# gaozhihan/PreDiff

Hardware: AMD Instinct MI355X
Metric: denoising_steps_per_sec (higher is better)
Workload: dtype bf16; 1 GPU; SEVIR-LR 7->6 x128x128 (latent 13x16x16, C 256/512, depth [4,4], axial), DDIM-50 eta=0, no knowledge alignment (BASELINE.json configs[1]); trajectories_per_gpu=64, global_trajectories=64, sampler=ddim50, hip_graph=True, lanes=2, trajectories_per_launch=32, parallelism=ensemble-shard x1

## Files before the change

### prediff_amd/csrc/igemm.hip

```cpp
#include <type_traits>
#include "common.h"
#include "igemm_epilogue.h"

namespace PD_NS {

__device__ __attribute__((aligned(64))) uint32_t g_pd_zero_page[32];

#ifndef PD_BIG_TILE_DEFAULT
#define PD_BIG_TILE_DEFAULT 1
#endif

#define BLDS16(rsrc, ldsptr, voff, soff) \
  __builtin_amdgcn_raw_ptr_buffer_load_lds((rsrc), (__attribute__((address_space(3))) void*)(ldsptr), 16, (voff), (soff), 0, 0)
#define PD_OOB 0xffffff00u

template <int N>
__device__ __forceinline__ void wait_vmcnt() {
  asm volatile("s_waitcnt vmcnt(%0)" ::"n"(N) : "memory");
}

template <int BM, int BN, int BK, int NS, bool SPLIT, int KIND, int OCC = 2, int ESLAB = 1>
__global__ void __launch_bounds__(256, OCC) igemm_kernel(const pd_igemm_args p) {
#if defined(__HIP_DEVICE_COMPILE__)
  constexpr int ROWB = BK * 2;
  constexpr int CPR = ROWB / 16;
  constexpr int RPI = 256 / CPR;
  constexpr int A_TILE = BM * ROWB;
  constexpr int B_TILE = BN * ROWB;
  constexpr int NP = SPLIT ? 2 : 1;
  constexpr int STAGE = (A_TILE + B_TILE) * NP;
  constexpr int AI = BM / RPI, BI = BN / RPI;
  constexpr int LPS = (AI + BI) * NP;
  constexpr int KSUB = BK / 32;
  extern __shared__ __attribute__((aligned(16))) char smem[];

  const int tid = threadIdx.x;
  const int lane = tid & 63;
  const int wave = __builtin_amdgcn_readfirstlane(tid >> 6);

  const int tiles_n = (p.N + BN - 1) / BN;
  const int tiles_m = (p.M + BM - 1) / BM;
  const int nt = tiles_m * tiles_n;
  int t;
  {
    const int bid = blockIdx.x, xcd = bid & 7, q = nt >> 3, r = nt & 7;
    t = (xcd < r ? xcd * (q + 1) : r * (q + 1) + (xcd - r) * q) + (bid >> 3);
  }
  const int m0 = (t / tiles_n) * BM;
  const int n0 = (t % tiles_n) * BN;
  const int bz = blockIdx.z;

  const auto rA = __builtin_amdgcn_make_buffer_rsrc((void*)(p.A + (int64_t)bz * p.a_batch_stride), 0, p.a_bytes, 0x00020000);
  const auto rW = __builtin_amdgcn_make_buffer_rsrc((void*)(p.W + (int64_t)bz * p.w_batch_stride), 0, p.w_bytes, 0x00020000);
  const auto rAlo = __builtin_amdgcn_make_buffer_rsrc((void*)((SPLIT ? p.A_lo : p.A) + (int64_t)bz * p.a_batch_stride), 0, p.a_bytes, 0x00020000);
  const auto rWlo = __builtin_amdgcn_make_buffer_rsrc((void*)((SPLIT ? p.W_lo : p.W) + (int64_t)bz * p.w_batch_stride), 0, p.w_bytes, 0x00020000);

  const int srow = tid / CPR;
  const int spos = tid % CPR;
  const int schunk = (CPR == 8) ? (spos ^ ((srow >> 1) & 7)) : (spos ^ ((srow >> 2) & 3));
  int vt0[AI], vh0[AI], vw0[AI];
  uint32_t abase[AI];
  uint32_t aoff[AI];
#pragma unroll
  for (int i = 0; i < AI; ++i) {
    const int m = m0 + i * RPI + srow;
    if (KIND == 0) {
      aoff[i] = m < p.M ? ((uint32_t)m * (uint32_t)p.lda + schunk * 8) * 2u : PD_OOB;
    } else {
      const int hw_o = p.Ho * p.Wo, thw_o = p.To * hw_o;
      const bool ok = m < p.M;
      const int mm = ok ? m : 0;
      const int b = mm / thw_o, r1 = mm - b * thw_o;
      const int ot = r1 / hw_o, r2 = r1 - ot * hw_o;
      const int oh = r2 / p.Wo, ow = r2 - oh * p.Wo;
      vt0[i] = ok ? ot * p.st - p.pt : -(1 << 20);
      vh0[i] = oh * p.sh - p.ph;
      vw0[i] = ow * p.sw - p.pw;
      abase[i] = (uint32_t)b * (uint32_t)(p.Ti * p.Hi * p.Wi);
    }
  }
  uint32_t woff[BI];
#pragma unroll
  for (int i = 0; i < BI; ++i) {
    const int n = n0 + i * RPI + srow;
    woff[i] = n < p.N ? ((uint32_t)n * (uint32_t)p.ldw + schunk * 8) * 2u : PD_OOB;
  }
  const int kchunks = p.Cin / BK;
  const int nk = (p.debug_flags & 1) ? 0 : p.taps * kchunks;
  const int vT = p.vT > 0 ? p.vT : p.Ti * p.ut, vH = p.vH > 0 ? p.vH : p.Hi * p.uh, vW = p.vW > 0 ? p.vW : p.Wi * p.uw;
  const int khw = p.KH * p.KW;

  auto set_tap = [&](int tap) {
    if (p.w_fold > 0 && tap >= p.w_fold) tap -= p.w_fold;
    const int kt = tap / khw, r = tap - kt * khw;
    const int kh = r / p.KW, kw = r - kh * p.KW;
#pragma unroll
    for (int i = 0; i < AI; ++i) {
      const int vt = vt0[i] + kt, vh = vh0[i] + kh, vw = vw0[i] + kw;
      const bool ok = (unsigned)vt < (unsigned)vT && (unsigned)vh < (unsigned)vH && (unsigned)vw < (unsigned)vW;
      const int it = p.ut == 2 ? vt >> 1 : vt, ih = p.uh == 2 ? vh >> 1 : vh, iw = p.uw == 2 ? vw >> 1 : vw;
      aoff[i] = ok ? ((abase[i] + (uint32_t)((it * p.Hi + ih) * p.Wi + iw)) * (uint32_t)p.lda + schunk * 8) * 2u : PD_OOB;
    }
  };

  auto issue = [&](int stage, int ks) {
    const int tap = ks / kchunks, kc = ks - tap * kchunks;
    if (KIND != 0 && kc == 0) set_tap(tap);
    char* sbase = smem + stage * STAGE;
    const int ka = kc * (BK * 2);
    const int kw = (int)(((int64_t)tap * p.w_tap_stride + kc * BK) * 2);
#pragma unroll
    for (int i = 0; i < AI; ++i) {
      char* dst = sbase + (i * 256 + wave * 64) * 16;
      BLDS16(rA, dst, aoff[i], ka);
      if (SPLIT) BLDS16(rAlo, dst + A_TILE, aoff[i], ka);
    }
#pragma unroll
    for (int i = 0; i < BI; ++i) {
      char* dst = sbase + A_TILE * NP + (i * 256 + wave * 64) * 16;
      BLDS16(rW, dst, woff[i], kw);
      if (SPLIT) BLDS16(rWlo, dst + B_TILE, woff[i], kw);
    }
  };

  constexpr int TM16 = BM / 32, TN16 = BN / 32;
  f32x4 acc[TM16][TN16];
#pragma unroll
  for (int i = 0; i < TM16; ++i)
#pragma unroll
    for (int j = 0; j < TN16; ++j)
#pragma unroll
      for (int r = 0; r < 4; ++r) acc[i][j][r] = 0.f;

  const int wr = wave >> 1, wc = wave & 1;
  const int l16 = lane & 15, lg = lane >> 4;
  const int swz = (CPR == 8) ? ((l16 >> 1) & 7) : ((l16 >> 2) & 3);
  const int a_row_b = (wr * (BM / 2) + l16) * ROWB;
  const int b_row_b = (wc * (BN / 2) + l16) * ROWB;

  constexpr int D = NS - 1;
#pragma unroll
  for (int s0 = 0; s0 < D; ++s0)
    if (s0 < nk) issue(s0, s0);
  int stage = 0;
  for (int ks = 0; ks < nk; ++ks) {
    const int younger = min(D - 1, nk - ks - 1);
    if (D >= 3 && younger == 2) wait_vmcnt<2 * LPS>();
    else if (D >= 2 && younger == 1) wait_vmcnt<LPS>();
    else wait_vmcnt<0>();
    __builtin_amdgcn_s_barrier();
    if (ks + D < nk) issue((stage + D) % NS, ks + D);
    const char* sA = smem + stage * STAGE;
    const char* sB = sA + A_TILE * NP;
#pragma unroll
    for (int kk = 0; kk < KSUB; ++kk) {
      const int pos = ((kk * 4 + lg) ^ swz) * 16;
      op8 a[TM16], b[TN16], al[TM16], bl[TN16];
#pragma unroll
      for (int i = 0; i < TM16; ++i) {
        a[i] = *(const op8*)(sA + a_row_b + i * 16 * ROWB + pos);
        if (SPLIT) al[i] = *(const op8*)(sA + A_TILE + a_row_b + i * 16 * ROWB + pos);
      }
#pragma unroll
      for (int j = 0; j < TN16; ++j) {
        b[j] = *(const op8*)(sB + b_row_b + j * 16 * ROWB + pos);
        if (SPLIT) bl[j] = *(const op8*)(sB + B_TILE + b_row_b + j * 16 * ROWB + pos);
      }
#pragma unroll
      for (int i = 0; i < TM16; ++i)
#pragma unroll
        for (int j = 0; j < TN16; ++j) {
          if (SPLIT) {
            acc[i][j] = mfma_16x16x32(al[i], b[j], acc[i][j]);
            acc[i][j] = mfma_16x16x32(a[i], bl[j], acc[i][j]);
          }
          acc[i][j] = mfma_16x16x32(a[i], b[j], acc[i][j]);
        }
    }
    stage = stage + 1 == NS ? 0 : stage + 1;
  }

  constexpr int WM = BM / 2, WN = BN / 2;
  constexpr int WNS = WN / ESLAB;
  constexpr int TNS = TN16 / ESLAB;
  float* sC = (float*)smem + wave * (WM * WNS);
#pragma unroll
  for (int js = 0; js < ESLAB; ++js) {
    __syncthreads();
#pragma unroll
    for (int i = 0; i < TM16; ++i)
#pragma unroll
      for (int j = 0; j < TNS; ++j)
#pragma unroll
        for (int r = 0; r < 4; ++r)
          sC[(i * 16 + 4 * lg + r) * WNS + j * 16 + l16] = acc[i][js * TNS + j][r];
    __syncthreads();
    igemm_epilogue<WM, WNS>(p, sC, lane, m0 + wr * WM, p.M, n0 + wc * WN + js * WNS, bz);
  }
#endif
}

template <int BM, int BN, int BK, int NS, bool SPLIT, int KIND, int OCC = 2, int ESLAB = 1>
static int launch_igemm(const pd_igemm_args& a, hipStream_t s) {
  constexpr int stage = (BM + BN) * BK * 2 * (SPLIT ? 2 : 1);
  constexpr int epi = 4 * (BM / 2) * (BN / 2) * 4 / ESLAB;
  constexpr int lds = NS * stage > epi ? NS * stage : epi;
  static bool attr_set_dev[PD_MAX_DEVICES];
  bool& attr_set = attr_set_dev[pd_cur_device()];
  if (!attr_set) {
    hipError_t e = hipFuncSetAttribute((const void*)igemm_kernel<BM, BN, BK, NS, SPLIT, KIND, OCC, ESLAB>,
                                       hipFuncAttributeMaxDynamicSharedMemorySize, lds);
    if (e != hipSuccess) {
      pd_set_error("pd_igemm: hipFuncSetAttribute(%d) failed: %s", lds, hipGetErrorString(e));
      return PD_ERR_LAUNCH;
    }
    attr_set = true;
  }
  const int tiles = ((a.M + BM - 1) / BM) * ((a.N + BN - 1) / BN);
  dim3 grid(tiles, 1, a.nbatch > 0 ? a.nbatch : 1);
  hipLaunchKernelGGL((igemm_kernel<BM, BN, BK, NS, SPLIT, KIND, OCC, ESLAB>), grid, dim3(256), lds, s, a);
  PD_CHECK_LAUNCH();
  return PD_OK;
}

template <bool SPLIT, int KIND>
static int dispatch_igemm(const pd_igemm_args& a, int tile, hipStream_t s) {
  switch (tile) {
    case 1: return launch_igemm<128, 128, 64, 2, SPLIT, KIND>(a, s);
    case 2: return launch_igemm<64, 64, 64, 2, SPLIT, KIND>(a, s);
    case 3: return launch_igemm<128, 128, 32, 4, SPLIT, KIND>(a, s);
    case 4: return launch_igemm<128, 128, 64, 3, SPLIT, KIND>(a, s);
    case 5: return launch_igemm<128, 128, 32, 2, SPLIT, KIND, (SPLIT ? 2 : 4), 2>(a, s);
    case 6: return launch_igemm<128, 128, 32, 3, SPLIT, KIND, (SPLIT ? 2 : 3), 2>(a, s);
    case 8: return launch_igemm<128, 64, 64, 2, SPLIT, KIND>(a, s);
    case 9: return launch_igemm<64, 128, 64, 2, SPLIT, KIND>(a, s);
    default: pd_set_error("pd_igemm: unknown tile config %d", tile); return PD_ERR_ARG;
  }
}

bool pd_igemm256_supported(const pd_igemm_args& a, int kind);
int pd_igemm256_launch(const pd_igemm_args& a, int kind, hipStream_t s);

int pd_igemm256_ksplit(const pd_igemm_args& a, int kind);
int pd_igemm256_launch_splitk(const pd_igemm_args& a, int kind, hipStream_t s);

#if !PD_IS_F16
extern "C" int pd_f16_igemm(const pd_igemm_args*, pd_stream_t);
#endif

extern "C" int PD_ENTRY(igemm)(const pd_igemm_args* pa, pd_stream_t stream) {
  PD_CHECK_ARG(pa != nullptr, "pd_igemm: null args");
  PD_FORWARD_F16(pa->operand == PD_OPERAND_F16, pd_f16_igemm(pa, stream));
  pd_igemm_args a = *pa;
  PD_CHECK_ARG(!PD_IS_F16 || (!a.split && !a.fp8 && !a.out_bf16_lo), "pd_igemm: IEEE-half operands: no hi/lo split, no e4m3 operands");
  const int min_k_256 = a.min_k_256 > 0 ? a.min_k_256 : a.split ? 256 : 1024;
  PD_CHECK_ARG(a.A && a.W, "pd_igemm: A/W null");
  PD_CHECK_ARG(a.M > 0 && a.N > 0 && a.taps > 0, "pd_igemm: bad M/N/taps (%d,%d,%d)", a.M, a.N, a.taps);
  PD_CHECK_ARG(a.Cin > 0 && (a.Cin & 63) == 0, "pd_igemm: Cin=%d must be a positive multiple of 64 (zero padded)", a.Cin);
  PD_CHECK_ARG((a.lda & 7) == 0 && (a.ldw & 7) == 0, "pd_igemm: lda/ldw must be multiples of 8 (16 B rows)");
  PD_CHECK_ARG(a.w_fold >= 0 && (a.w_fold == 0 || (!a.split && !a.fp8 && a.taps == 2 * a.w_fold)),
               "pd_igemm: w_fold = %d needs taps = 2 w_fold (W_hi slabs then W_lo slabs), no hi/lo split, no e4m3 operands", a.w_fold);
  PD_CHECK_ARG((a.w_fold ? a.w_fold : a.taps) == a.KT * a.KH * a.KW, "pd_igemm: taps != KT*KH*KW");
  PD_CHECK_ARG((int64_t)a.B * a.To * a.Ho * a.Wo == a.M, "pd_igemm: M != B*To*Ho*Wo");
  PD_CHECK_ARG((a.ut == 1 || a.ut == 2) && (a.uh == 1 || a.uh == 2) && (a.uw == 1 || a.uw == 2), "pd_igemm: bad upsample");
  if (a.fp8) {
    PD_CHECK_ARG((a.Cin & 127) == 0 && (a.lda & 15) == 0 && (a.ldw & 15) == 0, "pd_igemm: fp8 operands need Cin %% 128 == 0 and lda/ldw %% 16 == 0");
    PD_CHECK_ARG(!a.split && a.nbatch <= 1, "pd_igemm: fp8 operands: no hi/lo split, no batch");
  }
  {
    const int eb = a.fp8 ? 1 : 2;
    const int64_t abytes = (int64_t)a.B * a.Ti * a.Hi * a.Wi * (int64_t)a.lda * eb;
    const int64_t wbytes = ((int64_t)(a.taps - 1) * a.w_tap_stride + (int64_t)a.N * a.ldw) * eb;
    PD_CHECK_ARG(abytes < 0xfffffe00ll && wbytes < 0xfffffe00ll, "pd_igemm: operand larger than a 4 GiB buffer descriptor");
    a.a_bytes = (uint32_t)abytes;
    a.w_bytes = (uint32_t)wbytes;
  }
  PD_CHECK_ARG(!a.split || (a.A_lo && a.W_lo), "pd_igemm: split needs A_lo and W_lo");
  PD_CHECK_ARG(!a.rowvec || a.rows_per_sample > 0, "pd_igemm: rowvec needs rows_per_sample");
  PD_CHECK_ARG(a.out_f32 || a.out_bf16, "pd_igemm: no output");
  hipStream_t s = (hipStream_t)stream;
  a.vec_epilogue = ((a.N & 3) == 0) && (!a.out_f32 || (a.ld_out & 3) == 0) && (!a.out_bf16 || (a.ld_outb & 3) == 0) &&
                   (!a.residual || (a.ld_res & 3) == 0) && (!a.rowvec || (a.ld_rowvec & 3) == 0) &&
                   (!a.mul || (a.ld_mul & 3) == 0) && (((uintptr_t)a.out_f32 | (uintptr_t)a.residual | (uintptr_t)a.rowvec |
                   (uintptr_t)a.mul) & 15) == 0 && (((uintptr_t)a.out_bf16 | (uintptr_t)a.out_bf16_lo) & 7) == 0 &&
                   ((a.out_batch_stride | a.outb_batch_stride | a.res_batch_stride) & 3) == 0;
  if (a.vec_epilogue && !a.out_f32 && a.out_bf16 && (a.N & 7) == 0 && (a.ld_outb & 7) == 0 && (a.outb_batch_stride & 7) == 0 &&
      (((uintptr_t)a.out_bf16 | (uintptr_t)a.out_bf16_lo) & 15) == 0)
    a.vec_epilogue = 2;
  if (a.out_fp8_log2 > 0) {
    PD_CHECK_ARG(a.vec_epilogue == 2 && !a.out_bf16_lo && !a.split && a.out_fp8_log2 <= 16,
                 "pd_igemm: an e4m3 output needs the 8-column vector epilogue (out_bf16 only, N %% 8 == 0, ld_outb %% 8 == 0, 16 B aligned), no split");
  }
  int tile = a.tile;
  const bool pointwise = (a.taps == 1 || a.w_fold == 1) && a.st == 1 && a.sh == 1 && a.sw == 1 && a.pt == 0 && a.ph == 0 && a.pw == 0 && a.ut == 1 &&
                         a.uh == 1 && a.uw == 1 && a.Ti == a.To && a.Hi == a.Ho && a.Wi == a.Wo && a.vT <= 0 && a.vH <= 0 && a.vW <= 0;
  const int kind = pointwise ? 0 : ((a.KT == 1 && a.Ti == 1 && a.To == 1) ? 1 : 2);
  a.ksplit = 1;
#if !PD_IS_F16
  if (a.fp8) {
    if (!pd_igemm256_supported(a, kind) || kind == 1) {
      pd_set_error("pd_igemm: fp8 operands are built for row-wise linear layers and stride-1, un-upsampled Conv3d launches only");
      return PD_ERR_UNSUPPORTED;
    }
    const int ks = (a.tile == 0 && !a.disable_256 && a.out_fp8_log2 <= 0) ? pd_igemm256_ksplit(a, kind) : 0;
    if (ks >= 2) {
      a.ksplit = ks;
      return pd_igemm256_launch_splitk(a, kind, s);
    }
    return pd_igemm256_launch(a, kind, s);
  }
#endif
  if (tile == 0 && !a.disable_256) {
    const int ks = pd_igemm256_ksplit(a, kind);
    if (ks >= 2) {
      a.ksplit = ks;
      return pd_igemm256_launch_splitk(a, kind, s);
    }
  }
  if (tile == 0) {
    const int64_t t128 = (int64_t)((a.M + 127) / 128) * ((a.N + 127) / 128) * (a.nbatch > 0 ? a.nbatch : 1);
    tile = t128 >= 192 ? ((!a.split && (int64_t)a.taps * a.Cin <= 256) ? 5 : PD_BIG_TILE_DEFAULT) : 2;
    if (tile == PD_BIG_TILE_DEFAULT && !a.disable_256 && (int64_t)a.taps * a.Cin >= min_k_256 && pd_igemm256_supported(a, kind)) {
      const int64_t t256 = (int64_t)((a.M + 255) / 256) * ((a.N + 255) / 256) * (a.nbatch > 0 ? a.nbatch : 1);
      const int64_t ncu = pd_num_cus();
      const int64_t r128 = a.split ? (t128 + ncu - 1) / ncu : (t128 + 2 * ncu - 1) / (2 * ncu), r256 = (t256 + ncu - 1) / ncu;
      if (a.split ? r256 * 11 <= r128 * 5 : r256 * 33 <= r128 * 20) tile = 7;
    }
  }
  if (a.split && tile == 4) tile = 1;
  if (tile == 7) {
    if (pd_igemm256_supported(a, kind)) return pd_igemm256_launch(a, kind, s);
    tile = PD_BIG_TILE_DEFAULT;
  }
#if !PD_IS_F16
  if (a.split) {
    if (kind == 0) return dispatch_igemm<true, 0>(a, tile, s);
    if (kind == 1) return dispatch_igemm<true, 1>(a, tile, s);
    return dispatch_igemm<true, 2>(a, tile, s);
  }
#endif
  if (kind == 0) return dispatch_igemm<false, 0>(a, tile, s);
  if (kind == 1) return dispatch_igemm<false, 1>(a, tile, s);
  return dispatch_igemm<false, 2>(a, tile, s);
}

}
```

Baseline: 1540 steps/s.

## Add halo-tiled 3x3x3 conv kernel reusing LDS frame tiles across spatial taps

```diff
diff --git a/prediff_amd/csrc/conv3d_halo.hip b/prediff_amd/csrc/conv3d_halo.hip
--- /dev/null
+++ b/prediff_amd/csrc/conv3d_halo.hip
@@ -0,0 +1,250 @@
+#include <algorithm>
+#include "common.h"
+#include "igemm_epilogue.h"
+
+namespace PD_NS {
+
+#define BLDS16(rsrc, ldsptr, voff, soff) \
+  __builtin_amdgcn_raw_ptr_buffer_load_lds((rsrc), (__attribute__((address_space(3))) void*)(ldsptr), 16, (voff), (soff), 0, 0)
+#define PD_OOB 0xffffff00u
+#define VMCNT(n) asm volatile("s_waitcnt vmcnt(" #n ")" ::: "memory")
+#define PHASE_SYNC()                   \
+  __builtin_amdgcn_sched_barrier(0);   \
+  __builtin_amdgcn_s_barrier();        \
+  __builtin_amdgcn_sched_barrier(0)
+
+namespace {
+constexpr int FW = 16;
+constexpr int HW = FW + 2;
+constexpr int HROWS = HW * HW;
+constexpr int PLROWS = 336;
+constexpr int PLANE = PLROWS * 16;
+constexpr int HALO = 8 * PLANE;
+constexpr int NPIECE = HALO / 1024;
+constexpr int WHT = 128 * 128;
+constexpr int WBUF = 2 * WHT;
+constexpr int W_OFF = 2 * HALO;
+constexpr int HALO_LDS = W_OFF + 2 * WBUF;
+static_assert(PLANE % 256 == 0 && HALO % 1024 == 0 && PLROWS >= HROWS, "halo plane layout");
+static_assert(HALO_LDS >= 8 * 128 * 32 * 4, "the epilogue stages 128 KB of accumulators in the operand buffers");
+
+struct FragH {
+  op8 v[2];
+};
+}
+
+__global__ void __launch_bounds__(512) conv3d_halo_kernel(const pd_igemm_args p) {
+#if defined(__HIP_DEVICE_COMPILE__)
+  extern __shared__ __attribute__((aligned(16))) char smem[];
+  const int tid = threadIdx.x;
+  const int lane = tid & 63;
+  const int wave = __builtin_amdgcn_readfirstlane(tid >> 6);
+  const int wr = wave >> 2, wc = wave & 3;
+
+  const int tiles_n = (p.N + 255) >> 8;
+  const int tiles_m = p.M >> 8;
+  const int nt = tiles_m * tiles_n;
+  int t;
+  {
+    const int bid = blockIdx.x, xcd = bid & 7, q = nt >> 3, r = nt & 7;
+    t = (xcd < r ? xcd * (q + 1) : r * (q + 1) + (xcd - r) * q) + (bid >> 3);
+  }
+  const int tm = t / tiles_n;
+  const int m0 = tm << 8;
+  const int n0 = (t % tiles_n) << 8;
+
+  const auto rA = __builtin_amdgcn_make_buffer_rsrc((void*)p.A, 0, p.a_bytes, 0x00020000);
+  const auto rW = __builtin_amdgcn_make_buffer_rsrc((void*)p.W, 0, p.w_bytes, 0x00020000);
+
+  const int srow = tid >> 3, spos = tid & 7;
+  const uint32_t w_sel = (uint32_t)(spos ^ ((srow >> 1) & 7)) * 16u;
+  uint32_t woff[2][2];
+#pragma unroll
+  for (int hh = 0; hh < 2; ++hh)
+#pragma unroll
+    for (int i = 0; i < 2; ++i) {
+      const int n = n0 + hh * 128 + i * 64 + srow;
+      woff[hh][i] = n < p.N ? ((uint32_t)n * (uint32_t)p.ldw) * 2u + w_sel : PD_OOB;
+    }
+  uint32_t hoff[6];
+#pragma unroll
+  for (int n = 0; n < 6; ++n) {
+    const int cell = (wave + 8 * n) * 64 + lane;
+    const int s = cell / PLROWS, r = cell - s * PLROWS;
+    const int hr = r / HW, hc = r - hr * HW;
+    const bool ok = cell < 8 * PLROWS && r < HROWS && hr >= 1 && hr <= FW && hc >= 1 && hc <= FW;
+    hoff[n] = ok ? (uint32_t)((hr - 1) * FW + (hc - 1)) * (uint32_t)p.lda * 2u + (uint32_t)s * 16u : PD_OOB;
+  }
+
+  const int kchunks = p.Cin >> 6;
+  const int ot = tm % p.To;
+  const bool dense = (p.debug_flags & 8) != 0;
+  const int kt_lo = dense ? 0 : max(0, 1 - ot), kt_hi = dense ? 2 : min(2, p.Ti - ot);
+  const int ngroups = (p.debug_flags & 1) ? 0 : kchunks * (kt_hi - kt_lo + 1);
+  const uint32_t frame_b = 256u * (uint32_t)p.lda * 2u;
+  const uint32_t w_tap_b = (uint32_t)p.w_tap_stride * 2u;
+
+  int h_c = 0, h_kt = kt_lo, w_c = 0, w_kt = kt_lo;
+  uint32_t w_off = (uint32_t)(kt_lo * 9) * w_tap_b;
+  int h_soff = 0;
+  uint32_t h_mask = 0;
+  char* const h_dst = smem + wave * 1024;
+  char* const w_dst = smem + W_OFF + wave * 1024;
+  auto next_halo = [&]() {
+    const int it = ot - 1 + h_kt;
+    const bool ok = (unsigned)it < (unsigned)p.Ti;
+    h_soff = __builtin_amdgcn_readfirstlane(ok ? (int)((uint32_t)(tm - 1 + h_kt) * frame_b + (uint32_t)h_c * 128u) : 0);
+    h_mask = ok ? 0u : PD_OOB;
+    if (++h_kt > kt_hi) { h_kt = kt_lo; ++h_c; }
+  };
+  auto issue_h = [&](int n, int buf) { BLDS16(rA, h_dst + buf * HALO + n * 8192, hoff[n] | h_mask, h_soff); };
+  auto next_w_group = [&]() {
+    if (++w_kt > kt_hi) { w_kt = kt_lo; ++w_c; }
+    w_off = (uint32_t)(w_kt * 9) * w_tap_b + (uint32_t)w_c * 128u;
+  };
+  auto issue_w = [&](int buf) {
+    const int so = __builtin_amdgcn_readfirstlane((int)w_off);
+    char* dst = w_dst + buf * WBUF;
+    BLDS16(rW, dst, woff[0][0], so);
+    BLDS16(rW, dst + 64 * 128, woff[0][1], so);
+    BLDS16(rW, dst + WHT, woff[1][0], so);
+    BLDS16(rW, dst + WHT + 64 * 128, woff[1][1], so);
+    w_off += w_tap_b;
+  };
+
+  f32x4 acc[8][4];
+#pragma unroll
+  for (int i = 0; i < 8; ++i)
+#pragma unroll
+    for (int j = 0; j < 4; ++j)
+#pragma unroll
+      for (int r = 0; r < 4; ++r) acc[i][j][r] = 0.f;
+
+  const int l16 = lane & 15, lg = lane >> 4;
+  const int swz = (l16 >> 1) & 7;
+  const int a_rd = (wr * (8 * HW) + l16) * 16 + lg * PLANE;
+  const int b_rd = W_OFF + (wc >> 1) * WHT + ((wc & 1) * 64 + l16) * 128;
+
+  if (ngroups > 0) {
+    next_halo();
+    if (wave < 2) issue_h(5, 0);
+#pragma unroll
+    for (int n = 0; n < 5; ++n) issue_h(n, 0);
+    issue_w(0);
+    issue_w(1);
+    VMCNT(4);
+  }
+  __builtin_amdgcn_s_barrier();
+  if (wr == 1) __builtin_amdgcn_s_barrier();
+  __builtin_amdgcn_sched_barrier(0);
+
+  FragH a[4], b0[2], b1[2];
+#define LOAD_B(f, base) \
+  (f).v[0] = *(const op8*)((base) + ((lg ^ swz) * 16)); (f).v[1] = *(const op8*)((base) + (((4 + lg) ^ swz) * 16))
+#define LOAD_A(f, base) \
+  (f).v[0] = *(const op8*)(base); (f).v[1] = *(const op8*)((base) + 4 * PLANE)
+#define QUAD16(R0, C0, bfrag)                                                                               \
+  _Pragma("unroll") for (int ks = 0; ks < 2; ++ks)                                                          \
+    _Pragma("unroll") for (int i = 0; i < 4; ++i)                                                           \
+      _Pragma("unroll") for (int c = 0; c < 2; ++c)                                                         \
+        acc[(R0) + i][(C0) + c] = mfma_16x16x32(a[i].v[ks], bfrag[c].v[ks], acc[(R0) + i][(C0) + c]);
+
+  int wcur = 0;
+  auto group = [&](auto has_next_t, int g) {
+    constexpr bool has_next = decltype(has_next_t)::value;
+    const int hnxt = (g & 1) ^ 1;
+    const char* sA = smem + (g & 1) * HALO + a_rd;
+    if (has_next) next_halo();
+#pragma unroll
+    for (int j = 0; j < 9; ++j) {
+      const int shift = ((j / 3) * HW + (j % 3)) * 16;
+      const char* sB = smem + wcur * WBUF + b_rd;
+#pragma unroll
+      for (int c = 0; c < 2; ++c) { LOAD_B(b0[c], sB + c * (16 * 128)); }
+#pragma unroll
+      for (int i = 0; i < 4; ++i) { LOAD_A(a[i], sA + shift + i * (HW * 16)); }
+#pragma unroll
+      for (int c = 0; c < 2; ++c) { LOAD_B(b1[c], sB + (2 + c) * (16 * 128)); }
+      if (j >= 1 && j <= 5 && has_next) {
+        if (j == 1 && wave < 2) issue_h(5, hnxt);
+        issue_h(j - 1, hnxt);
+      }
+      PHASE_SYNC();
+      __builtin_amdgcn_s_setprio(1);
+      QUAD16(0, 0, b0)
+      QUAD16(0, 2, b1)
+      __builtin_amdgcn_s_setprio(0);
+      PHASE_SYNC();
+#pragma unroll
+      for (int i = 0; i < 4; ++i) { LOAD_A(a[i], sA + shift + (4 + i) * (HW * 16)); }
+      if (j <= 6 || has_next) {
+        if (j == 7) next_w_group();
+        issue_w(wcur);
+        if (j >= 1 && j <= 5 && has_next) {
+          VMCNT(5);
+        } else {
+          VMCNT(4);
+        }
+      } else {
+        VMCNT(0);
+      }
+      PHASE_SYNC();
+      __builtin_amdgcn_s_setprio(1);
+      QUAD16(4, 2, b1)
+      QUAD16(4, 0, b0)
+      __builtin_amdgcn_s_setprio(0);
+      PHASE_SYNC();
+      wcur ^= 1;
+    }
+  };
+  for (int g = 0; g + 1 < ngroups; ++g) group(std::true_type{}, g);
+  if (ngroups > 0) group(std::false_type{}, ngroups - 1);
+#undef QUAD16
+#undef LOAD_A
+#undef LOAD_B
+  if (wr == 0) __builtin_amdgcn_s_barrier();
+  if (p.debug_flags & 2) return;
+
+  float* sC = (float*)smem + wave * (128 * 32);
+  const int m_base = m0 + wr * 128;
+  const int m_end = min(p.M, m_base + 128);
+#pragma unroll
+  for (int js = 0; js < 2; ++js) {
+    __syncthreads();
+#pragma unroll
+    for (int i = 0; i < 8; ++i)
+#pragma unroll
+      for (int c = 0; c < 2; ++c)
+#pragma unroll
+        for (int r = 0; r < 4; ++r) sC[(i * 16 + 4 * lg + r) * 32 + c * 16 + l16] = acc[i][js * 2 + c][r];
+    __syncthreads();
+    igemm_epilogue<128, 32>(p, sC, lane, m_base, m_end, n0 + wc * 64 + js * 32, 0);
+  }
+#endif
+}
+
+bool pd_conv3d_halo_supported(const pd_igemm_args& a, int kind) {
+  if (kind != 2 || a.split || a.fp8 || a.w_fold > 0 || a.nbatch > 1) return false;
+  if (a.KT != 3 || a.KH != 3 || a.KW != 3 || a.pt != 1 || a.ph != 1 || a.pw != 1) return false;
+  if (a.st != 1 || a.sh != 1 || a.sw != 1 || a.ut != 1 || a.uh != 1 || a.uw != 1 || a.vT > 0 || a.vH > 0 || a.vW > 0) return false;
+  return a.Hi == FW && a.Wi == FW && a.Ho == FW && a.Wo == FW && a.Ti == a.To;
+}
+
+int pd_conv3d_halo_launch(const pd_igemm_args& a, hipStream_t s) {
+  static bool attr_set_dev[PD_MAX_DEVICES];
+  bool& attr_set = attr_set_dev[pd_cur_device()];
+  if (!attr_set) {
+    hipError_t e = hipFuncSetAttribute((const void*)conv3d_halo_kernel, hipFuncAttributeMaxDynamicSharedMemorySize, HALO_LDS);
+    if (e != hipSuccess) {
+      pd_set_error("pd_igemm: hipFuncSetAttribute(%d) failed: %s", HALO_LDS, hipGetErrorString(e));
+      return PD_ERR_LAUNCH;
+    }
+    attr_set = true;
+  }
+  const int tiles = (a.M / 256) * ((a.N + 255) / 256);
+  hipLaunchKernelGGL(conv3d_halo_kernel, dim3(tiles, 1, 1), dim3(512), HALO_LDS, s, a);
+  PD_CHECK_LAUNCH();
+  return PD_OK;
+}
+
+}
diff --git a/prediff_amd/csrc/igemm.hip b/prediff_amd/csrc/igemm.hip
--- a/prediff_amd/csrc/igemm.hip
+++ b/prediff_amd/csrc/igemm.hip
@@ -243,6 +243,9 @@
 
 int pd_igemm256_ksplit(const pd_igemm_args& a, int kind);
 int pd_igemm256_launch_splitk(const pd_igemm_args& a, int kind, hipStream_t s);
+
+bool pd_conv3d_halo_supported(const pd_igemm_args& a, int kind);
+int pd_conv3d_halo_launch(const pd_igemm_args& a, hipStream_t s);
 
 #if !PD_IS_F16
 extern "C" int pd_f16_igemm(const pd_igemm_args*, pd_stream_t);
@@ -325,7 +328,12 @@
       const int64_t ncu = pd_num_cus();
       const int64_t r128 = a.split ? (t128 + ncu - 1) / ncu : (t128 + 2 * ncu - 1) / (2 * ncu), r256 = (t256 + ncu - 1) / ncu;
       if (a.split ? r256 * 11 <= r128 * 5 : r256 * 33 <= r128 * 20) tile = 7;
-    }
+      if (tile == 7 && !(a.debug_flags & 16) && pd_conv3d_halo_supported(a, kind)) tile = 10;
+    }
+  }
+  if (tile == 10) {
+    if (pd_conv3d_halo_supported(a, kind)) return pd_conv3d_halo_launch(a, s);
+    tile = 7;
   }
   if (a.split && tile == 4) tile = 1;
   if (tile == 7) {
```

After: 1588 steps/s, median of 6. 1.03x the previous value.
